# hongfz16/Garment4D

Hardware: AMD Instinct MI355X
Metric: point-cloud frames/s (FPS+ball_query+SA-MLP+LBS), B=8 N=8192 (higher is better)
Workload: dtype f32

## Files before the change

### garment4d_amd/csrc/ball_grid.hip

```cpp
#include <cstdlib>

#include "g4d_common.h"
#include "ball_grid_build.h"

namespace g4d {

__global__ void __launch_bounds__(kBuildThreads) ball_grid_build_kernel(int n, int cmax, int budget, float cell_req, const float *__restrict__ xyz_all,
                                                                       unsigned char *__restrict__ ws_all, size_t ws_stride) {
    ball_grid_build_body(n, cmax, budget, cell_req, xyz_all, ws_all, ws_stride, blockIdx.x);
}

struct BgArgs {
    float radius2[4];
    int nsample[4];
    int *idx[4];
};

__device__ __forceinline__ int query_cell(float v, float lo, float inv_c, int g) {
    const float u = floorf((v - lo) * inv_c);
    return (int)fminf(fmaxf(u, -2.f), (float)(g + 1));
}

template <int NS, int FM>
__global__ void __launch_bounds__(256) ball_grid_query_kernel(int n, int m, int qpw, const BgArgs a, const float *__restrict__ new_xyz_all,
                                                             const float *__restrict__ xyz_all, const unsigned char *__restrict__ ws_all,
                                                             size_t ws_stride, int cmax) {
    __shared__ int lst[4][NS][kCap];
    const int t = threadIdx.x, lane = t & 63;
    const int wave = __builtin_amdgcn_readfirstlane(t >> 6);
    const int b = blockIdx.y;
    const unsigned char *ws = ws_all + (size_t)b * ws_stride;
    const GridHdr *hdr = reinterpret_cast<const GridHdr *>(ws);
    const int *cellstart = reinterpret_cast<const int *>(ws + kGridHdrBytes);
    const float4 *sorted = reinterpret_cast<const float4 *>(ws + kGridHdrBytes + ((((size_t)cmax + 1) * 4 + 63) & ~(size_t)63));
    const float *xyz = xyz_all + (size_t)b * n * 3;
    const float lox = hdr->lox, loy = hdr->loy, loz = hdr->loz, inv_c = hdr->inv_c;
    const int gx = hdr->gx, gy = hdr->gy, gz = hdr->gz;
    const int ry = lane % 3 - 1, rz = (lane / 3) % 3 - 1;

    for (int qi = 0; qi < qpw; ++qi) {
        const int q = (blockIdx.x * 4 + wave) * qpw + qi;
        if (q >= m) break;
        const float *qp = new_xyz_all + ((size_t)b * m + q) * 3;
        const float qx = qp[0], qy = qp[1], qz = qp[2];
        const int cx = query_cell(qx, lox, inv_c, gx), cy = query_cell(qy, loy, inv_c, gy), cz = query_cell(qz, loz, inv_c, gz);
        const int x0 = max(cx - 1, 0), x1 = min(cx + 1, gx - 1);
        const int yy = cy + ry, zz = cz + rz;
        int s = 0, e = 0;
        if (lane < 9 && x0 <= x1 && yy >= 0 && yy < gy && zz >= 0 && zz < gz) {
            const int row = (zz * gy + yy) * gx;
            s = cellstart[row + x0];
            e = cellstart[row + x1 + 1];
        }
        int cum[10], off[9];
        cum[0] = 0;
#pragma unroll
        for (int r = 0; r < 9; ++r) {
            const int rs = __builtin_amdgcn_readlane(s, r), re = __builtin_amdgcn_readlane(e, r);
            off[r] = rs - cum[r];
            cum[r + 1] = cum[r] + (re - rs);
        }
        const int total = cum[9];
        int h[NS];
#pragma unroll
        for (int sc = 0; sc < NS; ++sc) h[sc] = 0;

        for (int j0 = 0; j0 < total; j0 += 4 * 64) {
            bool all_dense = true;
#pragma unroll
            for (int sc = 0; sc < NS; ++sc) all_dense &= h[sc] > kCap;
            if (all_dense) break;
            float4 p[4];
            bool valid[4];
#pragma unroll
            for (int u = 0; u < 4; ++u) {
                const int j = j0 + u * 64 + lane;
                valid[u] = j < total;
                int o = off[0];
#pragma unroll
                for (int r = 1; r < 9; ++r) o = (j >= cum[r]) ? off[r] : o;
                p[u] = sorted[valid[u] ? j + o : 0];
            }
#pragma unroll
            for (int u = 0; u < 4; ++u) {
                if (j0 + u * 64 >= total) break;
                const float d2 = dist2<FM>(qx - p[u].x, qy - p[u].y, qz - p[u].z);
#pragma unroll
                for (int sc = 0; sc < NS; ++sc) {
                    const bool hit = valid[u] && d2 < a.radius2[sc];
                    const unsigned long long mask = __builtin_amdgcn_ballot_w64(hit);
                    if (mask != 0ull) {
                        const int slot = h[sc] + (int)__builtin_amdgcn_mbcnt_hi((unsigned)(mask >> 32), __builtin_amdgcn_mbcnt_lo((unsigned)mask, 0u));
                        if (hit && slot < kCap) lst[wave][sc][slot] = __float_as_int(p[u].w);
                        h[sc] += __builtin_popcountll(mask);
                    }
                }
            }
        }

#pragma unroll
        for (int sc = 0; sc < NS; ++sc) {
            const int ns = a.nsample[sc];
            int *out = a.idx[sc] + ((size_t)b * m + q) * ns;
            const int hs = h[sc];
            if (hs == 0) {
                for (int l = lane; l < ns; l += 64) out[l] = 0;
            } else if (hs <= kCap) {
                int *L = lst[wave][sc];
                int hacc = hs;
                if (hs > ns) {
                    int v[kCapRegs];
#pragma unroll
                    for (int e = 0; e < kCapRegs; ++e) v[e] = (e * 64 + lane < hs) ? L[e * 64 + lane] : 0x7fffffff;
                    const int ne = (hs + 63) >> 6;
                    int lo = 0, hi = n;
                    while (lo < hi) {
                        const int mid = (lo + hi) >> 1;
                        int c = 0;
#pragma unroll
                        for (int e = 0; e < kCapRegs; ++e)
                            if (e < ne) c += __builtin_popcountll(__builtin_amdgcn_ballot_w64(v[e] < mid));
                        if (c >= ns) hi = mid; else lo = mid + 1;
                    }
                    int w = 0;
#pragma unroll
                    for (int e = 0; e < kCapRegs; ++e)
                        if (e < ne) {
                            const bool keep = v[e] < lo;
                            const unsigned long long mask = __builtin_amdgcn_ballot_w64(keep);
                            const int slot = w + (int)__builtin_amdgcn_mbcnt_hi((unsigned)(mask >> 32), __builtin_amdgcn_mbcnt_lo((unsigned)mask, 0u));
                            if (keep) L[slot] = v[e];
                            w += __builtin_popcountll(mask);
                        }
                    hacc = w;
                }
                int first = 0;
                for (int i0 = 0; i0 < hacc; i0 += 64) {
                    const int i = i0 + lane;
                    const int v = i < hacc ? L[i] : 0x7fffffff;
                    int rank = 0;
#pragma unroll 4
                    for (int j = 0; j < hacc; ++j) rank += (L[j] < v) ? 1 : 0;
                    if (i < hacc && rank < ns) out[rank] = v;
                    const unsigned long long z = __builtin_amdgcn_ballot_w64(i < hacc && rank == 0);
                    if (z != 0ull) first = __builtin_amdgcn_readlane(v, __builtin_ctzll(z));
                }
                for (int l = hacc + lane; l < ns; l += 64) out[l] = first;
            } else {
                const float r2 = a.radius2[sc];
                int cnt = 0, first = 0;
                for (int base = 0; base < n && cnt < ns; base += 64) {
                    const int k = base + lane;
                    const int kc = min(k, n - 1);
                    const float d2 = dist2<FM>(qx - xyz[kc * 3 + 0], qy - xyz[kc * 3 + 1], qz - xyz[kc * 3 + 2]);
                    const bool hit = k < n && d2 < r2;
                    const unsigned long long mask = __builtin_amdgcn_ballot_w64(hit);
                    if (mask != 0ull) {
                        if (cnt == 0) first = base + __builtin_ctzll(mask);
                        const int slot = cnt + (int)__builtin_amdgcn_mbcnt_hi((unsigned)(mask >> 32), __builtin_amdgcn_mbcnt_lo((unsigned)mask, 0u));
                        if (hit && slot < ns) out[slot] = k;
                        cnt += __builtin_popcountll(mask);
                    }
                }
                for (int l = cnt + lane; l < ns; l += 64) out[l] = first;
            }
        }
    }
}

__device__ __forceinline__ void nn3_insert_lex(float d, int k, float &b1, float &b2, float &b3, int &i1, int &i2, int &i3) {
    const bool lt1 = d < b1 || (d == b1 && k < i1), lt2 = d < b2 || (d == b2 && k < i2), lt3 = d < b3 || (d == b3 && k < i3);
    const float nb3 = lt2 ? b2 : (lt3 ? d : b3);
    const int ni3 = lt2 ? i2 : (lt3 ? k : i3);
    const float nb2 = lt1 ? b1 : (lt2 ? d : b2);
    const int ni2 = lt1 ? i1 : (lt2 ? k : i2);
    b1 = lt1 ? d : b1; i1 = lt1 ? k : i1;
    b2 = nb2; i2 = ni2; b3 = nb3; i3 = ni3;
}

template <int FM, bool STAGE>
__global__ void __launch_bounds__(256) three_nn_grid_kernel(int n, int m, const float *__restrict__ unknown_all,
                                                           const unsigned char *__restrict__ ws_all, size_t ws_stride, int cmax,
                                                           float *__restrict__ dist2_all, int *__restrict__ idx_all) {
    extern __shared__ __attribute__((aligned(16))) unsigned char nn_smem[];
    const int b = blockIdx.y;
    const int p = blockIdx.x * 256 + threadIdx.x;
    const unsigned char *ws = ws_all + (size_t)b * ws_stride;
    const GridHdr h = *reinterpret_cast<const GridHdr *>(ws);
    const int *cellstart = reinterpret_cast<const int *>(ws + kGridHdrBytes);
    const float4 *rec = reinterpret_cast<const float4 *>(ws + kGridHdrBytes + ((((size_t)cmax + 1) * 4 + 63) & ~(size_t)63));
    if constexpr (STAGE) {
        float4 *srec = reinterpret_cast<float4 *>(nn_smem);
        int *scell = reinterpret_cast<int *>(nn_smem + (size_t)m * 16);
        for (int k = threadIdx.x; k < m; k += 256) srec[k] = rec[k];
        for (int k = threadIdx.x; k <= h.ncells; k += 256) scell[k] = cellstart[k];
        __syncthreads();
        rec = srec;
        cellstart = scell;
    }
    const float *u = unknown_all + ((size_t)b * n + min(p, n - 1)) * 3;
    const float ux = u[0], uy = u[1], uz = u[2];
    const float INF = __builtin_inff();
    float b1 = INF, b2 = INF, b3 = INF;
    int i1 = 0, i2 = 0, i3 = 0;
    auto visit = [&](int k0, int k1) {
        int k = k0;
        for (; k + 1 < k1; k += 2) {
            const float4 r0 = rec[k], r1 = rec[k + 1];
            const float d0 = dist2<FM>(ux - r0.x, uy - r0.y, uz - r0.z);
            const float d1 = dist2<FM>(ux - r1.x, uy - r1.y, uz - r1.z);
            nn3_insert_lex(d0, __float_as_int(r0.w), b1, b2, b3, i1, i2, i3);
            nn3_insert_lex(d1, __float_as_int(r1.w), b1, b2, b3, i1, i2, i3);
        }
        if (k < k1) {
            const float4 r0 = rec[k];
            nn3_insert_lex(dist2<FM>(ux - r0.x, uy - r0.y, uz - r0.z), __float_as_int(r0.w), b1, b2, b3, i1, i2, i3);
        }
    };
    const float fx = (ux - h.lox) * h.inv_c, fy = (uy - h.loy) * h.inv_c, fz = (uz - h.loz) * h.inv_c;
    bool pending = true;
    const bool local = fx > -1.f && fx < (float)h.gx + 1.f && fy > -1.f && fy < (float)h.gy + 1.f && fz > -1.f && fz < (float)h.gz + 1.f;
    if (local) {
        const int cx = (int)floorf(fx), cy = (int)floorf(fy), cz = (int)floorf(fz);
        const float edge = h.inv_c > 0.f ? 1.0f / h.inv_c : INF;
        {
            const int x0 = max(cx - 1, 0), x1 = min(cx + 1, h.gx - 1);
            int rs[9], re[9];
#pragma unroll
            for (int q = 0; q < 9; ++q) {
                const int y = cy + (q % 3) - 1, z = cz + (q / 3) - 1;
                const bool ok = x0 <= x1 && y >= 0 && y < h.gy && z >= 0 && z < h.gz;
                const int row = ok ? (z * h.gy + y) * h.gx : 0;
                rs[q] = ok ? cellstart[row + x0] : 0;
                re[q] = ok ? cellstart[row + x1 + 1] : 0;
            }
#pragma unroll
            for (int q = 0; q < 9; ++q) visit(rs[q], re[q]);
            const float reach = edge * 0.99f;
            pending = !(b3 < reach * reach);
        }
        if (pending) {
            b1 = b2 = b3 = INF; i1 = i2 = i3 = 0;
            const int x0 = max(cx - 2, 0), x1 = min(cx + 2, h.gx - 1);
            if (x0 <= x1) {
                for (int dz = -2; dz <= 2; ++dz) {
                    const int z = cz + dz;
                    if (z < 0 || z >= h.gz) continue;
                    for (int dy = -2; dy <= 2; ++dy) {
                        const int y = cy + dy;
                        if (y < 0 || y >= h.gy) continue;
                        const int row = (z * h.gy + y) * h.gx;
                        visit(cellstart[row + x0], cellstart[row + x1 + 1]);
                    }
                }
            }
            const float reach = 2.f * edge * 0.99f;
            pending = !(b3 < reach * reach);
        }
    }
    if (pending) {
        b1 = b2 = b3 = INF; i1 = i2 = i3 = 0;
        visit(0, m);
    }
    if (p < n) {
        float *d2 = dist2_all + ((size_t)b * n + p) * 3;
        int *ix = idx_all + ((size_t)b * n + p) * 3;
        d2[0] = b1; d2[1] = b2; d2[2] = b3;
        ix[0] = i1; ix[1] = i2; ix[2] = i3;
    }
}

void grid_sorted_layout(int n, size_t *offset_bytes, size_t *stride_bytes) {
    *offset_bytes = kGridHdrBytes + ((((size_t)grid_cmax(n) + 1) * 4 + 63) & ~(size_t)63);
    *stride_bytes = grid_cloud_bytes(n);
}

int grid_build(int b, int n, float rmax, const float *xyz, void *ws, hipStream_t st, int budget) {
    const int cmax = grid_cmax(n);
    if (budget <= 0 || budget > cmax) budget = cmax;
    const size_t lds = ((size_t)cmax + 1) * 4 + 16 * 8 * 4;
    static unsigned long long attr = 0;
    if (const int rc = ensure_dynamic_lds(reinterpret_cast<const void *>(ball_grid_build_kernel), 160 * 1024 - 1024, attr, "g4d_ball_grid_build_f32"))
        return rc;
    hipLaunchKernelGGL(ball_grid_build_kernel, dim3(b), dim3(kBuildThreads), lds, st, n, cmax, budget, rmax > 0.f ? rmax * kCellSlack : 0.f, xyz,
                       reinterpret_cast<unsigned char *>(ws), grid_cloud_bytes(n));
    return check_launch("g4d_ball_grid_build_f32");
}

size_t grid_bytes_per_cloud(int n) { return grid_cloud_bytes(n); }
size_t grid_records_offset(int n) { return kGridHdrBytes + ((((size_t)grid_cmax(n) + 1) * 4 + 63) & ~(size_t)63); }

template <int NS, int FM>
static void grid_query_launch(dim3 grid, hipStream_t st, int n, int m, int qpw, const BgArgs &a, const float *new_xyz, const float *xyz,
                              const void *ws) {
    hipLaunchKernelGGL((ball_grid_query_kernel<NS, FM>), grid, dim3(256), 0, st, n, m, qpw, a, new_xyz, xyz,
                       reinterpret_cast<const unsigned char *>(ws), grid_cloud_bytes(n), grid_cmax(n));
}

static int grid_query(int b, int n, int m, int nscales, const float *radii, const int *nsamples, const float *new_xyz, const float *xyz,
                      int *const *idx, const void *ws, hipStream_t st) {
    BgArgs a = {};
    for (int s = 0; s < nscales; ++s) {
        a.radius2[s] = radii[s] * radii[s];
        a.nsample[s] = nsamples[s];
        a.idx[s] = idx[s];
    }
    const long long queries = (long long)b * m;
    int qpw = 1;
    while (qpw < 8 && queries / (qpw * 2) >= 32768) qpw <<= 1;
    static const int qpw_env = getenv("G4D_BG_QPW") ? atoi(getenv("G4D_BG_QPW")) : 0;
    if (qpw_env > 0) qpw = qpw_env;
    dim3 grid((unsigned)((m + 4 * qpw - 1) / (4 * qpw)), (unsigned)b);
    G4D_WITH_FM(distance_contraction(), switch (nscales) {
        case 1: grid_query_launch<1, FM>(grid, st, n, m, qpw, a, new_xyz, xyz, ws); break;
        case 2: grid_query_launch<2, FM>(grid, st, n, m, qpw, a, new_xyz, xyz, ws); break;
        case 3: grid_query_launch<3, FM>(grid, st, n, m, qpw, a, new_xyz, xyz, ws); break;
        default: grid_query_launch<4, FM>(grid, st, n, m, qpw, a, new_xyz, xyz, ws); break;
    })
    return check_launch("g4d_ball_grid_query_f32");
}

}

extern "C" size_t g4d_ball_grid_bytes(int b, int n) {
    if (b <= 0 || n <= 0) return 0;
    return (size_t)b * g4d::grid_cloud_bytes(n);
}

extern "C" int g4d_ball_grid_build_f32(int b, int n, float rmax, const float *xyz, void *grid, g4d_stream_t stream) {
    using namespace g4d;
    G4D_REQUIRE(b >= 0 && n >= 0 && b <= 65535, "g4d_ball_grid_build_f32: bad sizes (b=%d n=%d)", b, n);
    if (b == 0 || n == 0) return G4D_OK;
    G4D_REQUIRE(xyz && grid, "g4d_ball_grid_build_f32: null pointer");
    G4D_REQUIRE(rmax > 0.f && rmax < __builtin_inff(), "g4d_ball_grid_build_f32: rmax must be a positive finite radius");
    return grid_build(b, n, rmax, xyz, grid, reinterpret_cast<hipStream_t>(stream));
}

extern "C" int g4d_ball_grid_query_f32(int b, int n, int m, int nscales, const float *radii, const int *nsamples, const float *new_xyz,
                                       const float *xyz, int *const *idx, const void *grid, float grid_rmax, g4d_stream_t stream) {
    using namespace g4d;
    G4D_REQUIRE(b >= 0 && n >= 0 && m >= 0 && nscales >= 1 && nscales <= 4 && b <= 65535, "g4d_ball_grid_query_f32: bad sizes");
    G4D_REQUIRE(radii && nsamples && idx, "g4d_ball_grid_query_f32: null pointer");
    if (b == 0 || m == 0) return G4D_OK;
    hipStream_t st = reinterpret_cast<hipStream_t>(stream);
    for (int s = 0; s < nscales; ++s) {
        G4D_REQUIRE(nsamples[s] > 0 && idx[s], "g4d_ball_grid_query_f32: bad scale %d", s);
        G4D_REQUIRE(radii[s] <= grid_rmax, "g4d_ball_grid_query_f32: radius %g exceeds the radius the grid was built for (%g)", radii[s], grid_rmax);
        if (n == 0) {
            hipError_t e = hipMemsetAsync(idx[s], 0, sizeof(int) * (size_t)b * m * nsamples[s], st);
            if (e != hipSuccess) return (int)e;
        }
    }
    if (n == 0) return G4D_OK;
    G4D_REQUIRE(new_xyz && xyz && grid, "g4d_ball_grid_query_f32: null pointer");
    return grid_query(b, n, m, nscales, radii, nsamples, new_xyz, xyz, idx, grid, st);
}

extern "C" int g4d_ball_query_grid_f32(int b, int n, int m, int nscales, const float *radii, const int *nsamples, const float *new_xyz,
                                       const float *xyz, int *const *idx, void *grid, g4d_stream_t stream) {
    using namespace g4d;
    G4D_REQUIRE(nscales >= 1 && nscales <= 4 && radii, "g4d_ball_query_grid_f32: bad scales");
    float rmax = radii[0];
    for (int s = 1; s < nscales; ++s) rmax = radii[s] > rmax ? radii[s] : rmax;
    if (b > 0 && n > 0 && m > 0) {
        const int rc = g4d_ball_grid_build_f32(b, n, rmax, xyz, grid, stream);
        if (rc != G4D_OK) return rc;
    }
    return g4d_ball_grid_query_f32(b, n, m, nscales, radii, nsamples, new_xyz, xyz, idx, grid, rmax, stream);
}

extern "C" int g4d_three_nn_grid_f32(int b, int n, int m, const float *unknown, const float *known, float *dist2, int *idx, void *grid,
                                     g4d_stream_t stream) {
    using namespace g4d;
    G4D_REQUIRE(b >= 0 && n >= 0 && m >= 0 && b <= 65535, "g4d_three_nn_grid_f32: bad sizes (b=%d n=%d m=%d)", b, n, m);
    if ((long long)b * n == 0) return G4D_OK;
    G4D_REQUIRE(unknown && dist2 && idx, "g4d_three_nn_grid_f32: null pointer");
    if (m == 0) return g4d_three_nn_f32(b, n, m, unknown, known, dist2, idx, stream);
    G4D_REQUIRE(known && grid, "g4d_three_nn_grid_f32: null pointer (grid scratch = g4d_ball_grid_bytes(b, m))");
    hipStream_t st = reinterpret_cast<hipStream_t>(stream);
    static const int per_cell = [] { const char *e = getenv("G4D_NN_PER_CELL"); return e && atoi(e) > 0 ? atoi(e) : 1; }();
    if (const int rc = grid_build(b, m, 0.f, known, grid, st, m / per_cell > 8 ? m / per_cell : 8)) return rc;
    dim3 g((unsigned)((n + 255) / 256), (unsigned)b);
    const unsigned char *wsb = reinterpret_cast<const unsigned char *>(grid);
    if (m <= 2048) {
        const size_t lds = (size_t)m * 16 + ((size_t)grid_cmax(m) + 1) * 4;
        G4D_WITH_FM(distance_contraction(), hipLaunchKernelGGL((three_nn_grid_kernel<FM, true>), g, dim3(256), lds, st, n, m, unknown, wsb,
                                                              grid_cloud_bytes(m), grid_cmax(m), dist2, idx))
    } else {
        G4D_WITH_FM(distance_contraction(), hipLaunchKernelGGL((three_nn_grid_kernel<FM, false>), g, dim3(256), 0, st, n, m, unknown, wsb,
                                                              grid_cloud_bytes(m), grid_cmax(m), dist2, idx))
    }
    return check_launch("g4d_three_nn_grid_f32");
}
```

### garment4d_amd/csrc/ball_grid_build.h

```cpp
#pragma once
#include "g4d_common.h"

namespace g4d {

struct GridHdr {
    float lox, loy, loz, inv_c;
    int gx, gy, gz, ncells;
};

constexpr int kGridHdrBytes = 64;
constexpr int kBuildThreads = 1024;
constexpr int kCap = 512;
constexpr int kCapRegs = kCap / 64;
constexpr float kCellSlack = 1.01f;

__host__ __device__ inline int grid_cmax(int n) {
    int c = 512;
    while (c < n && c < 32768) c <<= 1;
    return c;
}
__host__ __device__ inline size_t grid_cloud_bytes(int n) {
    const size_t cells = ((size_t)grid_cmax(n) + 1) * 4;
    return kGridHdrBytes + ((cells + 63) & ~(size_t)63) + (size_t)n * 16;
}

__device__ __forceinline__ int cell_of(float v, float lo, float inv_c, int g) {
    const float u = fminf(fmaxf((v - lo) * inv_c, 0.f), (float)(g - 1));
    return (int)u;
}

__device__ __forceinline__ float wave_min_all(float v) {
#pragma unroll
    for (int o = 32; o > 0; o >>= 1) v = fminf(v, __shfl_xor(v, o));
    return v;
}
__device__ __forceinline__ float wave_max_all(float v) {
#pragma unroll
    for (int o = 32; o > 0; o >>= 1) v = fmaxf(v, __shfl_xor(v, o));
    return v;
}

__device__ __forceinline__ void ball_grid_build_body(int n, int cmax, int budget, float cell_req, const float *__restrict__ xyz_all,
                                                     unsigned char *__restrict__ ws_all, size_t ws_stride, int cloud) {
    extern __shared__ __attribute__((aligned(16))) int hist[];
    float *red = reinterpret_cast<float *>(hist + cmax + 1);
    const int t = threadIdx.x, lane = t & 63, wave = t >> 6;
    constexpr int T = kBuildThreads, W = T / 64;
    const float *xyz = xyz_all + (size_t)cloud * n * 3;
    unsigned char *ws = ws_all + (size_t)cloud * ws_stride;
    GridHdr *hdr = reinterpret_cast<GridHdr *>(ws);
    int *cellstart = reinterpret_cast<int *>(ws + kGridHdrBytes);
    float4 *sorted = reinterpret_cast<float4 *>(ws + kGridHdrBytes + ((((size_t)cmax + 1) * 4 + 63) & ~(size_t)63));
    const float INF = __builtin_inff();

    float lx = INF, ly = INF, lz = INF, hx = -INF, hy = -INF, hz = -INF;
    for (int k = t; k < n; k += T) {
        const float x = xyz[k * 3 + 0], y = xyz[k * 3 + 1], z = xyz[k * 3 + 2];
        if (fabsf(x) < INF) { lx = fminf(lx, x); hx = fmaxf(hx, x); }
        if (fabsf(y) < INF) { ly = fminf(ly, y); hy = fmaxf(hy, y); }
        if (fabsf(z) < INF) { lz = fminf(lz, z); hz = fmaxf(hz, z); }
    }
    lx = wave_min_all(lx); ly = wave_min_all(ly); lz = wave_min_all(lz);
    hx = wave_max_all(hx); hy = wave_max_all(hy); hz = wave_max_all(hz);
    if (lane == 0) { red[wave * 8 + 0] = lx; red[wave * 8 + 1] = ly; red[wave * 8 + 2] = lz;
                     red[wave * 8 + 3] = hx; red[wave * 8 + 4] = hy; red[wave * 8 + 5] = hz; }
    __syncthreads();
    for (int w = 0; w < W; ++w) {
        lx = fminf(lx, red[w * 8 + 0]); ly = fminf(ly, red[w * 8 + 1]); lz = fminf(lz, red[w * 8 + 2]);
        hx = fmaxf(hx, red[w * 8 + 3]); hy = fmaxf(hy, red[w * 8 + 4]); hz = fmaxf(hz, red[w * 8 + 5]);
    }
    if (!(lx <= hx)) { lx = 0.f; hx = 0.f; }
    if (!(ly <= hy)) { ly = 0.f; hy = 0.f; }
    if (!(lz <= hz)) { lz = 0.f; hz = 0.f; }
    float c = fmaxf(cell_req, 1e-30f);
    if (!(cell_req > 0.f)) {
        const float ex = fmaxf(hx - lx, 0.f), ey = fmaxf(hy - ly, 0.f), ez = fmaxf(hz - lz, 0.f);
        const float big = fmaxf(ex, fmaxf(ey, ez));
        const float vol = fmaxf(ex, big * 1e-3f) * fmaxf(ey, big * 1e-3f) * fmaxf(ez, big * 1e-3f);
        c = vol > 0.f && vol < INF ? 0.5f * cbrtf(vol / (float)budget) : 1e-30f;
        c = fmaxf(c, big * (1.0f / 1023.0f));
        if (!(c > 0.f && c < INF)) c = 1e-30f;
    }
    int gx, gy, gz;
    float inv_c;
    for (int it = 0; it < 400; ++it) {
        inv_c = 1.0f / c;
        const float fx = floorf((hx - lx) * inv_c), fy = floorf((hy - ly) * inv_c), fz = floorf((hz - lz) * inv_c);
        if (fx < 1024.f && fy < 1024.f && fz < 1024.f) {
            gx = (int)fx + 1; gy = (int)fy + 1; gz = (int)fz + 1;
            if ((long long)gx * gy * gz <= (long long)budget) break;
        }
        c *= 1.2599211f;
        gx = gy = gz = 1;
        inv_c = 0.f;
    }
    const int ncells = gx * gy * gz;
    __syncthreads();
    for (int i = t; i <= ncells; i += T) hist[i] = 0;
    __syncthreads();
    for (int k = t; k < n; k += T) {
        const int cell = (cell_of(xyz[k * 3 + 2], lz, inv_c, gz) * gy + cell_of(xyz[k * 3 + 1], ly, inv_c, gy)) * gx +
                         cell_of(xyz[k * 3 + 0], lx, inv_c, gx);
        atomicAdd(&hist[cell], 1);
    }
    __syncthreads();
    const int chunk = (ncells + T - 1) / T;
    const int c0 = min(t * chunk, ncells), c1 = min(c0 + chunk, ncells);
    int sum = 0;
    for (int i = c0; i < c1; ++i) sum += hist[i];
    int incl = sum;
#pragma unroll
    for (int o = 1; o < 64; o <<= 1) {
        const int up = __shfl_up(incl, o);
        if (lane >= o) incl += up;
    }
    int *wsum = reinterpret_cast<int *>(red);
    __syncthreads();
    if (lane == 63) wsum[wave] = incl;
    __syncthreads();
    int base = 0;
    for (int w = 0; w < wave; ++w) base += wsum[w];
    int run = base + incl - sum;
    for (int i = c0; i < c1; ++i) {
        const int v = hist[i];
        hist[i] = run;
        run += v;
    }
    if (t == 0) hist[ncells] = n;
    __syncthreads();
    for (int i = t; i <= ncells; i += T) cellstart[i] = hist[i];
    if (t == 0) {
        GridHdr h;
        h.lox = lx; h.loy = ly; h.loz = lz; h.inv_c = inv_c;
        h.gx = gx; h.gy = gy; h.gz = gz; h.ncells = ncells;
        *hdr = h;
    }
    __syncthreads();
    for (int k = t; k < n; k += T) {
        const float x = xyz[k * 3 + 0], y = xyz[k * 3 + 1], z = xyz[k * 3 + 2];
        const int cell = (cell_of(z, lz, inv_c, gz) * gy + cell_of(y, ly, inv_c, gy)) * gx + cell_of(x, lx, inv_c, gx);
        const int dst = atomicAdd(&hist[cell], 1);
        sorted[dst] = make_float4(x, y, z, __int_as_float(k));
    }
}


}
```

Measured before the change: 52170.

## Replace ball-query hit lists with per-wave LDS bitmaps over point indices

Reworks the grid ball-query so hits are recorded by atomically OR-ing bits into a per-wave shared-memory bitmap indexed by original point id, then extracting the first nsample indices in order with a DPP prefix scan. This removes the capped hit list, the rank/selection sort, and the brute-force fallback scan over all points for dense neighbourhoods. In exchange, each query pays for clearing and scanning the bitmap, and when n exceeds the bitmap span it re-walks the candidate cells once per span window. It also uses LDS atomics and dynamic shared memory up to 32KB per block, which may lower occupancy.

```diff
diff --git a/garment4d_amd/csrc/ball_grid.hip b/garment4d_amd/csrc/ball_grid.hip
--- a/garment4d_amd/csrc/ball_grid.hip
+++ b/garment4d_amd/csrc/ball_grid.hip
@@ -21,11 +21,22 @@
     return (int)fminf(fmaxf(u, -2.f), (float)(g + 1));
 }
 
+__device__ __forceinline__ int wave_prefix_incl(int v) {
+    v += __builtin_amdgcn_update_dpp(0, v, 0x111, 0xf, 0xf, false);
+    v += __builtin_amdgcn_update_dpp(0, v, 0x112, 0xf, 0xf, false);
+    v += __builtin_amdgcn_update_dpp(0, v, 0x114, 0xf, 0xf, false);
+    v += __builtin_amdgcn_update_dpp(0, v, 0x118, 0xf, 0xf, false);
+    v += __builtin_amdgcn_update_dpp(0, v, 0x142, 0xa, 0xf, false);
+    v += __builtin_amdgcn_update_dpp(0, v, 0x143, 0xc, 0xf, false);
+    return v;
+}
+
+__device__ __forceinline__ void wave_lds_fence() { __builtin_amdgcn_fence(__ATOMIC_ACQ_REL, "wavefront"); }
+
 template <int NS, int FM>
-__global__ void __launch_bounds__(256) ball_grid_query_kernel(int n, int m, int qpw, const BgArgs a, const float *__restrict__ new_xyz_all,
-                                                             const float *__restrict__ xyz_all, const unsigned char *__restrict__ ws_all,
-                                                             size_t ws_stride, int cmax) {
-    __shared__ int lst[4][NS][kCap];
+__global__ void __launch_bounds__(256) ball_grid_query_kernel(int n, int m, int qpw, int W, const BgArgs a, const float *__restrict__ new_xyz_all,
+                                                             const unsigned char *__restrict__ ws_all, size_t ws_stride, int cmax) {
+    extern __shared__ __attribute__((aligned(16))) unsigned bg_bits[];
     const int t = threadIdx.x, lane = t & 63;
     const int wave = __builtin_amdgcn_readfirstlane(t >> 6);
     const int b = blockIdx.y;
@@ -33,10 +44,18 @@
     const GridHdr *hdr = reinterpret_cast<const GridHdr *>(ws);
     const int *cellstart = reinterpret_cast<const int *>(ws + kGridHdrBytes);
     const float4 *sorted = reinterpret_cast<const float4 *>(ws + kGridHdrBytes + ((((size_t)cmax + 1) * 4 + 63) & ~(size_t)63));
-    const float *xyz = xyz_all + (size_t)b * n * 3;
     const float lox = hdr->lox, loy = hdr->loy, loz = hdr->loz, inv_c = hdr->inv_c;
     const int gx = hdr->gx, gy = hdr->gy, gz = hdr->gz;
     const int ry = lane % 3 - 1, rz = (lane / 3) % 3 - 1;
+    const int words = 64 * W;
+    const int span = words * 32;
+    unsigned *bm = bg_bits + (size_t)wave * NS * words;
+    uint4 *own = reinterpret_cast<uint4 *>(bm + lane * W);
+    const int W4 = W >> 2, words4 = words >> 2;
+#pragma unroll
+    for (int sc = 0; sc < NS; ++sc)
+        for (int k = 0; k < W4; ++k) own[sc * words4 + k] = make_uint4(0u, 0u, 0u, 0u);
+    wave_lds_fence();
 
     for (int qi = 0; qi < qpw; ++qi) {
         const int q = (blockIdx.x * 4 + wave) * qpw + qi;
@@ -61,110 +80,89 @@
             cum[r + 1] = cum[r] + (re - rs);
         }
         const int total = cum[9];
-        int h[NS];
-#pragma unroll
-        for (int sc = 0; sc < NS; ++sc) h[sc] = 0;
-
-        for (int j0 = 0; j0 < total; j0 += 4 * 64) {
-            bool all_dense = true;
-#pragma unroll
-            for (int sc = 0; sc < NS; ++sc) all_dense &= h[sc] > kCap;
-            if (all_dense) break;
-            float4 p[4];
-            bool valid[4];
-#pragma unroll
-            for (int u = 0; u < 4; ++u) {
-                const int j = j0 + u * 64 + lane;
-                valid[u] = j < total;
-                int o = off[0];
-#pragma unroll
-                for (int r = 1; r < 9; ++r) o = (j >= cum[r]) ? off[r] : o;
-                p[u] = sorted[valid[u] ? j + o : 0];
+        int got[NS], first[NS];
+        int *out[NS];
+#pragma unroll
+        for (int sc = 0; sc < NS; ++sc) {
+            got[sc] = 0;
+            first[sc] = 0;
+            out[sc] = a.idx[sc] + ((size_t)b * m + q) * a.nsample[sc];
+        }
+
+        for (int base = 0; base < n && total > 0; base += span) {
+            for (int j0 = 0; j0 < total; j0 += 4 * 64) {
+                float4 p[4];
+                bool valid[4];
+#pragma unroll
+                for (int u = 0; u < 4; ++u) {
+                    const int j = j0 + u * 64 + lane;
+                    valid[u] = j < total;
+                    int o = off[0];
+#pragma unroll
+                    for (int r = 1; r < 9; ++r) o = (j >= cum[r]) ? off[r] : o;
+                    p[u] = sorted[valid[u] ? j + o : 0];
+                }
+#pragma unroll
+                for (int u = 0; u < 4; ++u) {
+                    if (j0 + u * 64 >= total) break;
+                    const float d2 = dist2<FM>(qx - p[u].x, qy - p[u].y, qz - p[u].z);
+                    const unsigned rel = (unsigned)(__float_as_int(p[u].w) - base);
+                    const bool in = valid[u] && rel < (unsigned)span;
+                    const unsigned bit = 1u << (rel & 31u);
+#pragma unroll
+                    for (int sc = 0; sc < NS; ++sc)
+                        if (in && d2 < a.radius2[sc])
+                            (void)__hip_atomic_fetch_or(bm + sc * words + (rel >> 5), bit, __ATOMIC_RELAXED, __HIP_MEMORY_SCOPE_WAVEFRONT);
+                }
             }
-#pragma unroll
-            for (int u = 0; u < 4; ++u) {
-                if (j0 + u * 64 >= total) break;
-                const float d2 = dist2<FM>(qx - p[u].x, qy - p[u].y, qz - p[u].z);
-#pragma unroll
-                for (int sc = 0; sc < NS; ++sc) {
-                    const bool hit = valid[u] && d2 < a.radius2[sc];
-                    const unsigned long long mask = __builtin_amdgcn_ballot_w64(hit);
-                    if (mask != 0ull) {
-                        const int slot = h[sc] + (int)__builtin_amdgcn_mbcnt_hi((unsigned)(mask >> 32), __builtin_amdgcn_mbcnt_lo((unsigned)mask, 0u));
-                        if (hit && slot < kCap) lst[wave][sc][slot] = __float_as_int(p[u].w);
-                        h[sc] += __builtin_popcountll(mask);
+            wave_lds_fence();
+
+            bool more = false;
+#pragma unroll
+            for (int sc = 0; sc < NS; ++sc) {
+                const int ns = a.nsample[sc];
+                if (got[sc] >= ns) continue;
+                const uint4 *mine = own + sc * words4;
+                int cnt = 0, low = 0;
+                for (int k = 0; k < W4; ++k) {
+                    const uint4 v = mine[k];
+                    const unsigned w[4] = {v.x, v.y, v.z, v.w};
+#pragma unroll
+                    for (int c = 0; c < 4; ++c) {
+                        if (cnt == 0 && w[c] != 0u) low = base + (lane * W + k * 4 + c) * 32 + __builtin_ctz(w[c]);
+                        cnt += __builtin_popcount(w[c]);
                     }
                 }
+                const int incl = wave_prefix_incl(cnt);
+                const int hits = __builtin_amdgcn_readlane(incl, 63);
+                if (hits != 0) {
+                    if (got[sc] == 0) first[sc] = __builtin_amdgcn_readlane(low, __builtin_ctzll(__builtin_amdgcn_ballot_w64(cnt != 0)));
+                    int r = got[sc] + incl - cnt;
+                    for (int k = 0; k < W4 && r < ns; ++k) {
+                        const uint4 v = mine[k];
+                        unsigned w[4] = {v.x, v.y, v.z, v.w};
+#pragma unroll
+                        for (int c = 0; c < 4; ++c) {
+                            const int at = base + (lane * W + k * 4 + c) * 32;
+                            while (w[c] != 0u && r < ns) {
+                                out[sc][r++] = at + __builtin_ctz(w[c]);
+                                w[c] &= w[c] - 1u;
+                            }
+                        }
+                    }
+                    got[sc] += hits;
+                }
+                more |= got[sc] < ns;
             }
-        }
-
-#pragma unroll
-        for (int sc = 0; sc < NS; ++sc) {
-            const int ns = a.nsample[sc];
-            int *out = a.idx[sc] + ((size_t)b * m + q) * ns;
-            const int hs = h[sc];
-            if (hs == 0) {
-                for (int l = lane; l < ns; l += 64) out[l] = 0;
-            } else if (hs <= kCap) {
-                int *L = lst[wave][sc];
-                int hacc = hs;
-                if (hs > ns) {
-                    int v[kCapRegs];
-#pragma unroll
-                    for (int e = 0; e < kCapRegs; ++e) v[e] = (e * 64 + lane < hs) ? L[e * 64 + lane] : 0x7fffffff;
-                    const int ne = (hs + 63) >> 6;
-                    int lo = 0, hi = n;
-                    while (lo < hi) {
-                        const int mid = (lo + hi) >> 1;
-                        int c = 0;
-#pragma unroll
-                        for (int e = 0; e < kCapRegs; ++e)
-                            if (e < ne) c += __builtin_popcountll(__builtin_amdgcn_ballot_w64(v[e] < mid));
-                        if (c >= ns) hi = mid; else lo = mid + 1;
-                    }
-                    int w = 0;
-#pragma unroll
-                    for (int e = 0; e < kCapRegs; ++e)
-                        if (e < ne) {
-                            const bool keep = v[e] < lo;
-                            const unsigned long long mask = __builtin_amdgcn_ballot_w64(keep);
-                            const int slot = w + (int)__builtin_amdgcn_mbcnt_hi((unsigned)(mask >> 32), __builtin_amdgcn_mbcnt_lo((unsigned)mask, 0u));
-                            if (keep) L[slot] = v[e];
-                            w += __builtin_popcountll(mask);
-                        }
-                    hacc = w;
-                }
-                int first = 0;
-                for (int i0 = 0; i0 < hacc; i0 += 64) {
-                    const int i = i0 + lane;
-                    const int v = i < hacc ? L[i] : 0x7fffffff;
-                    int rank = 0;
-#pragma unroll 4
-                    for (int j = 0; j < hacc; ++j) rank += (L[j] < v) ? 1 : 0;
-                    if (i < hacc && rank < ns) out[rank] = v;
-                    const unsigned long long z = __builtin_amdgcn_ballot_w64(i < hacc && rank == 0);
-                    if (z != 0ull) first = __builtin_amdgcn_readlane(v, __builtin_ctzll(z));
-                }
-                for (int l = hacc + lane; l < ns; l += 64) out[l] = first;
-            } else {
-                const float r2 = a.radius2[sc];
-                int cnt = 0, first = 0;
-                for (int base = 0; base < n && cnt < ns; base += 64) {
-                    const int k = base + lane;
-                    const int kc = min(k, n - 1);
-                    const float d2 = dist2<FM>(qx - xyz[kc * 3 + 0], qy - xyz[kc * 3 + 1], qz - xyz[kc * 3 + 2]);
-                    const bool hit = k < n && d2 < r2;
-                    const unsigned long long mask = __builtin_amdgcn_ballot_w64(hit);
-                    if (mask != 0ull) {
-                        if (cnt == 0) first = base + __builtin_ctzll(mask);
-                        const int slot = cnt + (int)__builtin_amdgcn_mbcnt_hi((unsigned)(mask >> 32), __builtin_amdgcn_mbcnt_lo((unsigned)mask, 0u));
-                        if (hit && slot < ns) out[slot] = k;
-                        cnt += __builtin_popcountll(mask);
-                    }
-                }
-                for (int l = cnt + lane; l < ns; l += 64) out[l] = first;
-            }
-        }
+#pragma unroll
+            for (int sc = 0; sc < NS; ++sc)
+                for (int k = 0; k < W4; ++k) own[sc * words4 + k] = make_uint4(0u, 0u, 0u, 0u);
+            wave_lds_fence();
+            if (!more) break;
+        }
+#pragma unroll
+        for (int sc = 0; sc < NS; ++sc)
+            for (int l = got[sc] + lane; l < a.nsample[sc]; l += 64) out[sc][l] = first[sc];
     }
 }
 
@@ -290,15 +288,22 @@
 size_t grid_bytes_per_cloud(int n) { return grid_cloud_bytes(n); }
 size_t grid_records_offset(int n) { return kGridHdrBytes + ((((size_t)grid_cmax(n) + 1) * 4 + 63) & ~(size_t)63); }
 
+constexpr int kBitmapLds = 32 * 1024;
+static int bitmap_words_per_lane(int n, int nscales) {
+    const long long full = ((((long long)n + 31) / 32 + 63) / 64 + 3) & ~3ll;
+    const long long fit = (kBitmapLds / (4 * nscales * 64 * 4)) & ~3;
+    return (int)(full < fit ? full : fit);
+}
+
 template <int NS, int FM>
-static void grid_query_launch(dim3 grid, hipStream_t st, int n, int m, int qpw, const BgArgs &a, const float *new_xyz, const float *xyz,
-                              const void *ws) {
-    hipLaunchKernelGGL((ball_grid_query_kernel<NS, FM>), grid, dim3(256), 0, st, n, m, qpw, a, new_xyz, xyz,
+static void grid_query_launch(dim3 grid, hipStream_t st, int n, int m, int qpw, const BgArgs &a, const float *new_xyz, const void *ws) {
+    const int W = bitmap_words_per_lane(n, NS);
+    hipLaunchKernelGGL((ball_grid_query_kernel<NS, FM>), grid, dim3(256), (size_t)4 * NS * 64 * W * 4, st, n, m, qpw, W, a, new_xyz,
                        reinterpret_cast<const unsigned char *>(ws), grid_cloud_bytes(n), grid_cmax(n));
 }
 
-static int grid_query(int b, int n, int m, int nscales, const float *radii, const int *nsamples, const float *new_xyz, const float *xyz,
-                      int *const *idx, const void *ws, hipStream_t st) {
+static int grid_query(int b, int n, int m, int nscales, const float *radii, const int *nsamples, const float *new_xyz, int *const *idx,
+                      const void *ws, hipStream_t st) {
     BgArgs a = {};
     for (int s = 0; s < nscales; ++s) {
         a.radius2[s] = radii[s] * radii[s];
@@ -312,10 +317,10 @@
     if (qpw_env > 0) qpw = qpw_env;
     dim3 grid((unsigned)((m + 4 * qpw - 1) / (4 * qpw)), (unsigned)b);
     G4D_WITH_FM(distance_contraction(), switch (nscales) {
-        case 1: grid_query_launch<1, FM>(grid, st, n, m, qpw, a, new_xyz, xyz, ws); break;
-        case 2: grid_query_launch<2, FM>(grid, st, n, m, qpw, a, new_xyz, xyz, ws); break;
-        case 3: grid_query_launch<3, FM>(grid, st, n, m, qpw, a, new_xyz, xyz, ws); break;
-        default: grid_query_launch<4, FM>(grid, st, n, m, qpw, a, new_xyz, xyz, ws); break;
+        case 1: grid_query_launch<1, FM>(grid, st, n, m, qpw, a, new_xyz, ws); break;
+        case 2: grid_query_launch<2, FM>(grid, st, n, m, qpw, a, new_xyz, ws); break;
+        case 3: grid_query_launch<3, FM>(grid, st, n, m, qpw, a, new_xyz, ws); break;
+        default: grid_query_launch<4, FM>(grid, st, n, m, qpw, a, new_xyz, ws); break;
     })
     return check_launch("g4d_ball_grid_query_f32");
 }
@@ -353,7 +358,7 @@
     }
     if (n == 0) return G4D_OK;
     G4D_REQUIRE(new_xyz && xyz && grid, "g4d_ball_grid_query_f32: null pointer");
-    return grid_query(b, n, m, nscales, radii, nsamples, new_xyz, xyz, idx, grid, st);
+    return grid_query(b, n, m, nscales, radii, nsamples, new_xyz, idx, grid, st);
 }
 
 extern "C" int g4d_ball_query_grid_f32(int b, int n, int m, int nscales, const float *radii, const int *nsamples, const float *new_xyz,
diff --git a/garment4d_amd/csrc/ball_grid_build.h b/garment4d_amd/csrc/ball_grid_build.h
--- a/garment4d_amd/csrc/ball_grid_build.h
+++ b/garment4d_amd/csrc/ball_grid_build.h
@@ -10,8 +10,6 @@
 
 constexpr int kGridHdrBytes = 64;
 constexpr int kBuildThreads = 1024;
-constexpr int kCap = 512;
-constexpr int kCapRegs = kCap / 64;
 constexpr float kCellSlack = 1.01f;
 
 __host__ __device__ inline int grid_cmax(int n) {
```

Result: no change. 52640, median of 4 (+0.9%).
